# HuiGuanLab/Lite-MKD

Measured on AMD Instinct MI355X. Metric: episodes/sec (5-way 5-shot, 8x224^2 frames), higher is better.
Workload: dtype f32

## Files before the change

include/lmkd.h:

```cpp
#ifndef LMKD_H
#define LMKD_H
#ifdef __cplusplus
extern "C" {
#endif

int lmkd_abi_version(void);
const char* lmkd_last_error(void);
int lmkd_device_check(int device);
int lmkd_set_activation_dtype(int mode);
int lmkd_get_activation_dtype(void);

int lmkd_gemm_f32(char layA, char layB, int M, int N, int K, float alpha, const float* A, long lda, long sA,
                  const float* B, long ldb, long sB, float beta, float* C, long ldc, long sC, const float* bias,
                  int relu, int batch, void* stream);
int lmkd_gemm_set_mode(int mode);
int lmkd_gemm_set_tile(int t);
long lmkd_gemm_ticket_words(void);
int lmkd_gemm_f32_splitk(char layA, char layB, int M, int N, int K, float alpha, const float* A, long lda, long sA,
                         const float* B, long ldb, long sB, float beta, float* C, long ldc, long sC, const float* bias,
                         int relu, int batch, void* workspace, long ws_bytes, unsigned* tickets, void* stream);

long lmkd_conv2d_packed_weight_elems(int Cout, int Cin, int Cs, int KH, int KW, int mode);
int lmkd_conv2d_pack_weights(const float* w_oihw, float* wp, int Cout, int Cin, int Cs, int KH, int KW, int mode ,
                             void* stream);
// ... 5 lines not shown
  const void* x_words;
  const void* dy_words;
  void* out_words;
  const void* ref_words;
  int flags;
} lmkd_amax_desc;
#define LMKD_AMAX_FENCED 1
int lmkd_h2_fence_eval(const void* const* words, void* const* refs, int n, int* flags, void* stream);
long lmkd_conv_h2_fallbacks(void);
int lmkd_amax(const float* x, long n, void* word, void* stream);
long lmkd_amax_words(void);
long lmkd_conv2d_plane_elems(int ncols, int Kp);
long lmkd_conv_h2_launches(void);
int lmkd_conv2d_repack_multi(const float* const* ws, void* const* wfs, const int* dims, int n, void* stream);
int lmkd_conv2d_split_weights(const float* wp, void* wf, int ncols, int Kp, void* stream);
int lmkd_conv_get_compute_dtype(void);
int lmkd_conv_set_wgrad_planes(int on);
int lmkd_conv_set_patch(int on);
int lmkd_conv_set_stem_patch(int on);
int lmkd_conv_set_s2_patch(int on);
int lmkd_conv_set_wgrad_win16(int on);
int lmkd_conv_set_wgrad_stem(int on);
int lmkd_conv_set_wgrad_window(int on);
int lmkd_conv_set_patch16(int on);
int lmkd_conv_set_persistent(int on);
int lmkd_conv_set_xcd_mode(int mode);
int lmkd_conv_set_tile(int id);
int lmkd_conv2d_fwd(const float* x, const float* wp_fwd, float* y, float* stat_partial, int N, int H, int W, int Cs, int Cout,
                    int KH, int KW, int stride, int pad, void* stream);
int lmkd_conv2d_fwd_pre(const float* x_raw, const float* pre_stats, const float* wp_fwd, float* y, float* stat_partial, int N, int H,
                        int W, int Cs, int Cout, int KH, int KW, int stride, int pad, void* stream);
int lmkd_conv2d_fwd_bn(const float* x, const float* wp_fwd, float* y, const float* bn_stats, const float* res , int relu,
                       int N, int H, int W, int Cs, int Cout, int KH, int KW, int stride, int pad, void* stream,
                       const lmkd_amax_desc* amax );
int lmkd_conv2d_bwd_data(const float* dy, const float* wp_dgrad, float* dx, int N, int H, int W, int Cin, int Cout, int KH, int KW,
                         int stride, int pad, int accumulate, void* stream);
int lmkd_conv2d_bwd_data_bn_tiles(int N, int H, int W, int Cin, int Cout, int KH, int KW, int stride, int pad);
int lmkd_conv2d_bwd_data_bn(const float* dy, const float* wp_dgrad, float* dx, const float* bn_x, const float* bn_stats, float* part,
                            int N, int H, int W, int Cin, int Cout, int KH, int KW, int stride, int pad, void* stream);
long lmkd_conv2d_bwd_weight_workspace(int N, int H, int W, int Cs, int Cout, int KH, int KW, int stride, int pad);
int lmkd_conv2d_bwd_weight(const float* x, const float* dy, float* dw_oihw, float* workspace, long ws_bytes, int N, int H, int W,
                           int Cs, int Cin, int Cout, int KH, int KW, int stride, int pad, void* stream);
int lmkd_conv2d_bwd_weight_pre(const float* x_raw, const float* pre_stats, const float* dy, float* dw_oihw, float* workspace,
                               long ws_bytes, int N, int H, int W, int Cs, int Cin, int Cout, int KH, int KW, int stride, int pad,
                               void* stream);

// ... 236 lines not shown
```

lite-mkd_amd/_lib.py:

```python
import ctypes
import os
import re

from . import _audit

_HERE = os.path.dirname(os.path.abspath(__file__))
_ROOT = os.path.dirname(_HERE)
HEADER = os.path.join(_ROOT, "include", "lmkd.h")
LIB_PATH = os.environ.get("LMKD_LIB") or os.path.join(_HERE, "liblmkd_hip.so")

_CT = {
    "int": ctypes.c_int, "long": ctypes.c_long, "float": ctypes.c_float, "char": ctypes.c_char,
    "long long": ctypes.c_longlong, "unsigned long long": ctypes.c_ulonglong,
}


def parse_header(path=HEADER):
    txt = open(path).read()
    txt = re.sub(r"/\*.*?\*/", " ", txt, flags=re.S)
    protos = {}
    for m in re.finditer(r"\b(int|long|const char\s*\*)\s+(lmkd_\w+)\s*\(([^)]*)\)\s*;", txt):
        ret, name, args = m.group(1), m.group(2), m.group(3).strip()
        restype = ctypes.c_char_p if "char" in ret else _CT[ret]
        argtypes = []
# ... 7 lines not shown
                    ty = " ".join(toks[:-1])
                    argtypes.append(_CT[ty])
        protos[name] = (restype, argtypes)
    return protos


class _Lib:
    def __init__(self):
        if not os.path.exists(LIB_PATH):
            raise RuntimeError(
                "liblmkd_hip.so not found at %s: build it with `python lite-mkd_amd/build.py` "
                "(there is no CPU or PyTorch fallback for the hot path)" % LIB_PATH)
        import torch
        self.cdll = ctypes.CDLL(LIB_PATH)
        self.protos = parse_header()
        for name, (restype, argtypes) in self.protos.items():
            fn = getattr(self.cdll, name)
            fn.restype = restype
            fn.argtypes = argtypes
        if os.environ.get("LMKD_PATCH16"):
            self.cdll.lmkd_conv_set_patch16(int(os.environ["LMKD_PATCH16"]))
        if os.environ.get("LMKD_WGRAD_WINDOW"):
            self.cdll.lmkd_conv_set_wgrad_window(int(os.environ["LMKD_WGRAD_WINDOW"]))
        if os.environ.get("LMKD_CONV_PERSISTENT", "1") == "0":
            self.cdll.lmkd_conv_set_persistent(0)

    def last_error(self):
        return self.cdll.lmkd_last_error().decode()

    def call(self, name, *args):
        if _audit.ON:
            _audit.check(name)
        rc = getattr(self.cdll, name)(*args)
        if rc != 0:
            raise RuntimeError("%s failed (%d): %s" % (name, rc, self.last_error()))

    def value(self, name, *args):
        return getattr(self.cdll, name)(*args)


_lib = None


def lib():
    global _lib
    if _lib is None:
# ... 3 lines not shown
```

lite-mkd_amd/csrc/conv.hip:

```cpp
#include "gemm_core.h"
#include <atomic>
#include <mutex>

struct ConvGemmArgs {
  const float* src;
  const float* wpk;
  float* out;
  float* stat_partial;
  int N, Hs, Ws, Cs;
  int Hr, Wr, rows_per_class, tiles_per_class;
  int sh;
  int Ho, Wo, Co, omul;
  int Kp, cps, nclass;
  int n_rt, n_ct, xcd_mode;
  int taps_pm1;
  int grid_step;
  int grid_total;
  int same;
  int halo;
  int accum;
  const float* ep_stats;
  const float* ep_res;
  int ep_relu;
  const float* pre_stats;
// ... 1247 lines not shown
}
extern "C" int lmkd_conv2d_bwd_data_bn(const float* dy, const float* wd, float* dx, const float* bn_x, const float* bn_stats, float* part,
                                       int N, int H, int W, int Cin, int Cout, int KH, int KW, int stride, int pad, void* stream) {
  LMKD_REQUIRE(dy && wd && dx && bn_x && bn_stats && part, "lmkd_conv2d_bwd_data_bn: null pointer");
  LMKD_REQUIRE(aligned16(dy) && aligned16(wd) && aligned16(bn_x) && aligned16(bn_stats), "lmkd_conv2d_bwd_data_bn: operands must be 16-byte aligned");
  ConvGemmArgs a;
  if (const int rc = bwd_data_args(a, dy, wd, dx, N, H, W, Cin, Cout, KH, KW, stride, pad, 0)) return rc;
  a.bnb_x = bn_x; a.bnb_stats = bn_stats; a.stat_partial = part;
  const ConvPlan p = plan_dgrad(a);
  LMKD_REQUIRE(p.bnb_form, "lmkd_conv2d_bwd_data_bn: this launch has no fused form (lmkd_conv2d_bwd_data_bn_tiles returned 0)");
  return launch_conv(a, p, (hipStream_t)stream);
}

static int g_wgrad_planes = 1;
extern "C" int lmkd_conv_set_wgrad_planes(int on) { g_wgrad_planes = on ? 1 : 0; return LMKD_OK; }
static int g_wgrad_win16 = 1;
extern "C" int lmkd_conv_set_wgrad_win16(int on) { g_wgrad_win16 = on ? 1 : 0; return LMKD_OK; }
static int g_wgrad_window = 1;
extern "C" int lmkd_conv_set_wgrad_window(int on) { g_wgrad_window = on < 0 ? 0 : on; return LMKD_OK; }
static inline bool wgrad_win_eligible(int W, int Cs, int Cout, int KH, int KW, int stride, int pad) {
  return g_wgrad_window && g_wgrad_planes && conv_planes() && KH == 3 && KW == 3 && stride == 1 && pad == 1 &&
         Cs % 32 == 0 && 32 + 2 * (W + 1) <= 256;
}
static void wgrad_win_plan(int Mpix, int W, int Cs, int Cout, int* cob, int* splits, int* steps_per_split) {
  *cob = Cout >= 128 ? 4 : 2;
  const int tiles = cdiv(Cout, 32 * *cob) * (Cs / 32);
  const int steps = cdiv(Mpix, LMKD_BK);
  const int warm = cdiv(2 * (W + 1), LMKD_BK);
  const int resident = 256 * ((conv_nprod() >= 6 && *cob == 2) ? 2 : 8 / *cob);
  int sp = g_wgrad_window > 1 ? cdiv(g_wgrad_window, tiles)
                              : std::max((int)(((long)resident * steps + 19600L * 4 / *cob) / (39200L * 4 / *cob)), cdiv(128, tiles));
  const int cap = std::max(1, steps / (12 * warm));
  if (sp > cap) sp = cap;
  *steps_per_split = cdiv(steps, sp);
  *splits = cdiv(steps, *steps_per_split);
}

static void wgrad_plan(int Mpix, int Cout, int Kp, int* splits, int* steps_per_split, int* bm, int* bn, bool planes = false) {
  *bm = Cout <= 64 ? 64 : 128;
  *bn = (Kp % 128 == 0 && Kp >= 1024) ? 128 : 64;
  int per_cu = (*bm == 128 && *bn == 128) ? 2 : ((*bm == 64 && *bn == 64) ? 4 : 3);
  if (planes) {
    if (*bm == 64 && *bn == 128) *bn = 64;
    const int npl = conv_nprod() == 1 ? 1 : 3;
    const long lds = 1L * npl * LMKD_BK * ((*bm * 2 + 64) + (*bn * 2 + 64));
    per_cu = (int)(160 * 1024 / lds);
    if (per_cu > 4) per_cu = 4;
    if (per_cu < 1) per_cu = 1;
  }
  const int tiles = cdiv(Cout, *bm) * cdiv(Kp, *bn);
  const int steps = cdiv(Mpix, LMKD_BK);
  const int slots = 256 * per_cu;
  int best_sp = 1;
  double best_cost = 1e30;
// ... 14 lines not shown

static int g_wgrad_stem = 1;
extern "C" int lmkd_conv_set_wgrad_stem(int on) { g_wgrad_stem = on ? 1 : 0; return LMKD_OK; }
static int stem_wgrad_plan(int N, int H, int W, int Cs, int Cout, int KH, int KW, int stride, int pad, int* G) {
  if (!g_wgrad_stem || !g_wgrad_planes || conv_nprod(g_lmkd_act_bf16) < 6 || Cs != 4 || Cout != 64 || KH != 7 || KW != 7 || stride != 2 || pad != 3) return 0;
  const int Ho = conv_out(H, KH, stride, pad), Wo = conv_out(W, KW, stride, pad);
  if (Wo < 17 || Wo > 128 || W > 2 * Wo || Ho < 1) return 0;
  const int units = N * cdiv(Ho, 2);
  int g = std::max(1, 2048 / (2 * Wo));
  g = std::min(g, std::max(1, units / 256));
  *G = g;
  return cdiv(units, g);
}

enum class WgFam : unsigned char {
  Stem,
  Win16,
  Win,
  Planes,
  Tile,
};
struct WgradPlan {
  WgFam fam;
  bool pre, act16, smallc;
  int nprod;
  int bm, bn;
  int cob;
  int G;
  int splits, splits0, sps0, sps1, seg_pix0;
  int xcd;
  int grid;
  long need;
  long ws;
};

static long wgrad_workspace(int N, int H, int W, int Cs, int Cout, int KH, int KW, int stride, int pad) {
  const int Ho = conv_out(H, KH, stride, pad), Wo = conv_out(W, KW, stride, pad);
  const int Kp = KH * kw_padded(Cs, KW) * Cs;
  int G, splits, sps, bm, bn;
  if (const int slabs = stem_wgrad_plan(N, H, W, Cs, Cout, KH, KW, stride, pad, &G)) return (long)slabs * Cout * Kp * sizeof(float);
  wgrad_plan(N * Ho * Wo, Cout, Kp, &splits, &sps, &bm, &bn, conv_planes() && g_wgrad_planes);
  if (wgrad_win_eligible(W, Cs, Cout, KH, KW, stride, pad)) {
    int cob, wsplits, wsps;
    wgrad_win_plan(N * Ho * Wo, W, Cs, Cout, &cob, &wsplits, &wsps);
    splits = std::max(splits, wsplits);
  }
  return (long)splits * Cout * Kp * sizeof(float);
}

static WgradPlan plan_wgrad(int N, int H, int W, int Cs, int Cout, int KH, int KW, int stride, int pad, int seg_n0, bool pre, bool maxima) {
  WgradPlan p;
  memset(&p, 0, sizeof(p));
  const bool act16 = g_lmkd_act_bf16;
  const int Ho = conv_out(H, KH, stride, pad), Wo = conv_out(W, KW, stride, pad);
  const int Kp = KH * kw_padded(Cs, KW) * Cs, Mpix = N * Ho * Wo;
  p.pre = pre; p.act16 = act16; p.smallc = Cs == 4;
  p.ws = wgrad_workspace(N, H, W, Cs, Cout, KH, KW, stride, pad);
  if (seg_n0)
    p.ws = std::max(p.ws, wgrad_workspace(seg_n0, H, W, Cs, Cout, KH, KW, stride, pad) + wgrad_workspace(N - seg_n0, H, W, Cs, Cout, KH, KW, stride, pad));
  p.seg_pix0 = seg_n0 ? seg_n0 * Ho * Wo : Mpix;
  if (const int slabs = stem_wgrad_plan(N, H, W, Cs, Cout, KH, KW, stride, pad, &p.G)) {
    p.fam = WgFam::Stem;
    p.nprod = conv_nprod(false, maxima);
    p.splits = p.grid = slabs;
  } else if (wgrad_win_eligible(W, Cs, Cout, KH, KW, stride, pad)) {
    const bool w16 = g_wgrad_win16 && conv_nprod(act16) >= 6;
    p.fam = w16 ? WgFam::Win16 : WgFam::Win;
    p.nprod = w16 ? conv_nprod(false, maxima) : conv_nprod(act16);
    wgrad_win_plan(Mpix, W, Cs, Cout, &p.cob, &p.splits, &p.sps0);
    p.splits0 = p.splits;
    if (seg_n0) {
      int sp1, cob1;
      wgrad_win_plan(p.seg_pix0, W, Cs, Cout, &p.cob, &p.splits0, &p.sps0);
      wgrad_win_plan(Mpix - p.seg_pix0, W, Cs, Cout, &cob1, &sp1, &p.sps1);
      p.splits = p.splits0 + sp1;
    }
    p.grid = 8 * cdiv(p.splits, 8) * cdiv(Cout, 32 * p.cob) * (Cs / 32);
  } else {
    const bool planes = conv_planes() && g_wgrad_planes;
    p.fam = planes ? WgFam::Planes : WgFam::Tile;
    p.nprod = planes ? conv_nprod(act16, maxima && !p.smallc && !pre) : (conv_nprod() == 1 ? 1 : 0);
    wgrad_plan(Mpix, Cout, Kp, &p.splits, &p.sps0, &p.bm, &p.bn, planes);
    p.splits0 = p.splits;
    if (seg_n0) {
      int sp1, bm1, bn1;
      wgrad_plan(p.seg_pix0, Cout, Kp, &p.splits0, &p.sps0, &p.bm, &p.bn, planes);
      wgrad_plan(Mpix - p.seg_pix0, Cout, Kp, &sp1, &p.sps1, &bm1, &bn1, planes);
      p.splits = p.splits0 + sp1;
    }
    p.xcd = (g_xcd_mode != 0 && g_xcd_mode != 1 && p.splits >= 32) ? 1 : 0;
    p.grid = (p.xcd ? 8 * cdiv(p.splits, 8) : p.splits) * cdiv(Cout, p.bm) * cdiv(Kp, p.bn);
  }
  p.need = (long)p.splits * Cout * Kp * sizeof(float);
  return p;
}

template <int NPROD, int D, int RLC>
static void launch_stem_wgrad(const StemWgradArgs& w, dim3 grid, size_t lds, hipStream_t s) {
  lds_attr_once<stem_wgrad_kernel<NPROD, D, RLC>>(160 * 1024);
  hipLaunchKernelGGL((stem_wgrad_kernel<NPROD, D, RLC>), grid, dim3(512), lds, s, w);
}
template <int NPROD>
static void launch_stem_wgrad(const StemWgradArgs& w, dim3 grid, size_t lds, hipStream_t s) {
  const bool deep = cdiv(2 * w.Wo, 32) >= 6;
  if (deep && w.RL == 1856) launch_stem_wgrad<NPROD, 6, 1856>(w, grid, lds, s);
  else if (deep) launch_stem_wgrad<NPROD, 6, 0>(w, grid, lds, s);
  else launch_stem_wgrad<NPROD, 2, 0>(w, grid, lds, s);
}
template <int COB>
static void launch_wgrad_win(const WgradWinArgs& w, const WgradPlan& p, bool big, hipStream_t s) {
  const dim3 grid(p.grid);
  if (p.fam == WgFam::Win16) {
    constexpr int JW = COB == 2 ? 1 : 2;
    constexpr int NT = 64 * COB * (2 / JW);
    with_nprod<3, 6, 9>(p.nprod, [&](auto np) {
      if (big && p.pre) hipLaunchKernelGGL((conv_wgrad_win16_kernel<COB, np, 256, true, 9, JW>), grid, dim3(NT), 0, s, w);
      else if (big) hipLaunchKernelGGL((conv_wgrad_win16_kernel<COB, np, 256, false, 9, JW>), grid, dim3(NT), 0, s, w);
      else if (p.pre) hipLaunchKernelGGL((conv_wgrad_win16_kernel<COB, np, 128, true, 9, JW>), grid, dim3(NT), 0, s, w);
      else hipLaunchKernelGGL((conv_wgrad_win16_kernel<COB, np, 128, false, 9, JW>), grid, dim3(NT), 0, s, w);
    });
    return;
  }
  auto go = [&](auto np, auto a16, auto pre) {
    constexpr int NPROD = decltype(np)::value;
    constexpr bool A16 = decltype(a16)::value, PRE = decltype(pre)::value;
    constexpr int TPW = (COB == 2 && NPROD != 1) ? 5 : 9;
    constexpr int NT = 64 * COB * ((9 + TPW - 1) / TPW);
    if (big) hipLaunchKernelGGL((conv_wgrad_win_kernel<COB, NPROD, A16, 256, PRE, TPW>), grid, dim3(NT), 0, s, w);
    else hipLaunchKernelGGL((conv_wgrad_win_kernel<COB, NPROD, A16, 128, PRE, TPW>), grid, dim3(NT), 0, s, w);
  };
  using T = std::true_type;
  using F = std::false_type;
  if (p.act16) go(std::integral_constant<int, 1>{}, T{}, F{});
  else with_nprod<1, 6, 9>(p.nprod, [&](auto np) { if (p.pre) go(np, F{}, T{}); else go(np, F{}, F{}); });
// ... 46 lines not shown
  if (p.fam == WgFam::Stem) {
    LMKD_REQUIRE((long)Mpix * 64 * 4 < 0xffffffe0L && (long)N * H * W * 16 < 0xffffffe0L, "lmkd_conv2d_bwd_weight: tensor too large for 32-bit byte offsets");
    StemWgradArgs w;
    memset(&w, 0, sizeof(w));
    w.dy = dy; w.x = x; w.slab = workspace;
    w.h2_xw = amax_x; w.h2_dyw = amax_dy;
    w.N = N; w.H = H; w.W = W; w.Ho = Ho; w.Wo = Wo;
    w.upi = cdiv(Ho, 2); w.units = N * w.upi; w.G = p.G; w.slabs = p.splits;
    w.RL = 16 * Wo + 64;
    const size_t lds = (size_t)2 * 10 * 3 * w.RL + 2 * 3 * STEM_WG_APLANE;
    with_nprod<3, 6, 9>(p.nprod, [&](auto np) { launch_stem_wgrad<np>(w, dim3(p.grid), lds, s); });
    LMKD_CHECK_LAUNCH("stem_wgrad_kernel");
    if (Kp <= 256) {
      hipLaunchKernelGGL(wgrad_reduce_stem_kernel, dim3(Cout), dim3(256, 4), 0, s, (const float*)workspace, dw_oihw, p.splits, Cout, Cin, Cs, KH, KW,
                         KWp, Kp, accumulate);
    } else {
      launch_wgrad_reduce((const float*)workspace, dw_oihw, p.splits, Cout, Cin, Cs, KH, KW, KWp, Kp, accumulate, s);
    }
    LMKD_CHECK_LAUNCH("wgrad_reduce_kernel");
    return LMKD_OK;
  }
  if (p.fam == WgFam::Win16 || p.fam == WgFam::Win) {
    LMKD_REQUIRE((long)Mpix * std::max(Cs, Cout) * 4 < 2147483647L, "lmkd_conv2d_bwd_weight: tensor too large for 32-bit byte offsets");
    WgradWinArgs w;
    memset(&w, 0, sizeof(w));
    w.dy = dy; w.x = x; w.slab = workspace; w.pre_stats = pre_stats;
    w.h2_xw = amax_x; w.h2_dyw = amax_dy;
    w.N = N; w.H = H; w.W = W; w.Cs = Cs; w.Co = Cout; w.Kp = Kp; w.Mpix = Mpix;
    w.steps_total = cdiv(Mpix, LMKD_BK);
    w.splits = p.splits; w.steps_per_split = p.sps0;
    w.seg_pix0 = p.seg_pix0; w.seg_splits0 = p.splits0; w.sps1 = p.sps1;
    w.n_ct = cdiv(Cout, 32 * p.cob); w.n_it = Cs / 32;
    w.div_hw = make_fastdiv(H * W); w.div_w = make_fastdiv(W);
    const bool big = 32 + 2 * (W + 1) > 128;
    if (p.cob == 4) launch_wgrad_win<4>(w, p, big, s);
    else launch_wgrad_win<2>(w, p, big, s);
    LMKD_CHECK_LAUNCH("conv_wgrad_win_kernel");
    launch_wgrad_reduce((const float*)workspace, dw_oihw, p.splits, Cout, Cin, Cs, KH, KW, KWp, Kp, accumulate, s);
    LMKD_CHECK_LAUNCH("wgrad_reduce_kernel");
    return LMKD_OK;
  }
  WgradArgs a;
  memset(&a, 0, sizeof(a));
  a.dy = dy; a.x = x; a.slab = workspace; a.pre_stats = pre_stats;
  a.h2_xw = amax_x; a.h2_dyw = amax_dy;
  a.N = N; a.Hs = H; a.Ws = W; a.Cs = Cs;
  a.Ho = Ho; a.Wo = Wo; a.Co = Cout;
  a.stride = stride; a.pad = pad; a.KH = KH; a.KW = KW; a.KWp = KWp;
  a.Kp = Kp; a.Mpix = Mpix;
  a.steps_per_split = p.sps0;
  a.seg_pix0 = p.seg_pix0; a.seg_splits0 = p.splits0; a.sps1 = p.sps1;
  a.steps_total = cdiv(Mpix, LMKD_BK);
  a.div_hw = make_fastdiv(Ho * Wo); a.div_w = make_fastdiv(Wo);
  a.n_mt = cdiv(Cout, p.bm); a.n_jt = cdiv(Kp, p.bn); a.splits = p.splits;
  a.xcd_mode = p.xcd;
  const int bm = p.bm, bn = p.bn;
// ... 40 lines not shown
extern "C" int lmkd_conv2d_bwd_weight_acc(const float* x, const float* pre_stats, const float* dy, float* dw_oihw, float* workspace,
                                          long ws_bytes, int N, int H, int W, int Cs, int Cin, int Cout, int KH, int KW, int stride,
                                          int pad, void* stream) {
  return conv2d_bwd_weight_impl(x, pre_stats, dy, dw_oihw, workspace, ws_bytes, N, H, W, Cs, Cin, Cout, KH, KW, stride, pad, stream, 1);
}


extern "C" int lmkd_conv2d_bwd_weight_seg(const float* x, const float* pre_stats, const float* dy, float* dw_oihw, float* workspace, long ws_bytes,
                                          int N, int H, int W, int Cs, int Cin, int Cout, int KH, int KW, int stride, int pad, int accumulate,
                                          int seg_n0, void* stream, const lmkd_amax_desc* amax) {
  return conv2d_bwd_weight_impl(x, pre_stats, dy, dw_oihw, workspace, ws_bytes, N, H, W, Cs, Cin, Cout, KH, KW, stride, pad, stream, accumulate, seg_n0, amax);
}

extern "C" int lmkd_conv2d_plan(int kind, int N, int H, int W, int Cs, int Cin, int Cout, int KH, int KW, int stride, int pad,
                                int* info) {
  LMKD_REQUIRE(info && kind >= 0 && kind <= 2, "lmkd_conv2d_plan: kind must be 0 (forward), 1 (data gradient) or 2 (weight gradient)");
  LMKD_REQUIRE(N > 0 && H > 0 && W > 0 && Cout > 0 && KH > 0 && KW > 0 && stride > 0, "lmkd_conv2d_plan: bad shape");
  if (kind == 2) {
    const WgradPlan p = plan_wgrad(N, H, W, Cs, Cout, KH, KW, stride, pad, 0, false, false);
    info[1] = p.xcd; info[2] = p.splits; info[3] = p.grid;
    switch (p.fam) {
      case WgFam::Stem: info[0] = 14; info[4] = 2; break;
      case WgFam::Win16:
      case WgFam::Win: info[0] = p.cob == 4 ? 5 : 6; info[1] = 1; info[4] = 1; break;
      default: info[0] = (p.bm == 128 && p.bn == 128) ? 1 : (p.bm == 128 ? 2 : (p.bn == 128 ? 4 : 3)); info[4] = 0; break;
    }
    return LMKD_OK;
  }
  ConvGemmArgs a;
  if (kind == 0) fwd_geometry(a, N, H, W, Cs, Cout, KH, KW, stride, pad, 0);
  else dgrad_geometry(a, N, H, W, Cin, Cout, KH, KW, stride, pad, 0);
  const ConvPlan p = kind == 0 ? plan_fwd(a, KH, KW, pad) : plan_dgrad(a);
  info[0] = p.tile; info[1] = p.xcd; info[2] = p.nclass; info[3] = p.grid;
  info[4] = p.fam == ConvFam::Stem ? 2 : (p.fam == ConvFam::Patch || p.fam == ConvFam::Patch16 || p.fam == ConvFam::Patch1p ? 1 : 0);
  return LMKD_OK;
}
```

lite-mkd_amd/csrc/wgrad_win.h:

```cpp
#pragma once

struct WgradWinArgs {
  const float* dy;
  const float* x;
  float* slab;
  const float* pre_stats;
  int N, H, W, Cs, Co, Kp;
  int Mpix, steps_total, steps_per_split, splits;
  int n_ct, n_it;
  int seg_pix0, seg_splits0, sps1;
  FastDiv div_hw, div_w;
  const unsigned* h2_xw;
  const unsigned* h2_dyw;
};
template <int COB, int NPROD, bool ACT16, int R, bool PRE = false, int TPW = 9>
__global__ __launch_bounds__(64 * COB * ((9 + TPW - 1) / TPW)) void conv_wgrad_win_kernel(WgradWinArgs a) {
  constexpr int NPL = NPROD == 1 ? 1 : 3;
  static_assert(!ACT16 || (NPROD == 1 && !PRE), "bf16 tensors: one plane, no store-side arithmetic");
  constexpr int THREADS = 64 * COB * ((9 + TPW - 1) / TPW), BM = 32 * COB;
  constexpr int LDA = BM * 2 + 64, A_PLANE = LMKD_BK * LDA;
  constexpr int LDX = 64, X_PLANE = (R + 1) * LDX;
  constexpr int ESZ = ACT16 ? 2 : 4, EPL = ACT16 ? 8 : 4;
  constexpr int A_LPR = BM / EPL, A_RPP = THREADS / A_LPR, A_NI = (LMKD_BK + A_RPP - 1) / A_RPP;
  constexpr int X_LPR = 32 / EPL, X_RPP = THREADS / X_LPR, X_NI = (LMKD_BK + X_RPP - 1) / X_RPP;
// ... 150 lines not shown
            c = __builtin_amdgcn_mfma_f32_32x32x16_bf16(fa[g][1], fb[0], c, 0, 0, 0);
            c = __builtin_amdgcn_mfma_f32_32x32x16_bf16(fa[g][0], fb[0], c, 0, 0, 0);
          }
        }
        acc[ti] = c;
      }
      __syncthreads();
    }
  }

  float* C = a.slab + (long)z * a.Co * a.Kp;
#pragma unroll
  for (int ti = 0; ti < TPW; ++ti) {
    if (9 % TPW != 0 && tap0 + ti >= 9) break;
    const int col = (tap0 + ti) * a.Cs + ci0 + (lane & 31);
#pragma unroll
    for (int e = 0; e < 16; ++e) {
      const int row = co0 + cw * 32 + acc_row(e, lane);
      if (row < a.Co) C[(long)row * a.Kp + col] = acc[ti][e];
    }
  }
}

template <int COB, int NPROD, int R, bool PRE = false, int TPW = 9, int JW = 2>
__global__ __launch_bounds__(64 * COB * ((9 + TPW - 1) / TPW) * (2 / JW), JW == 2 ? 2 : 3) void conv_wgrad_win16_kernel(WgradWinArgs a) {
  static_assert(JW == 2 || (JW == 1 && TPW == 9), "the channel-block split exists for nine taps per wave");
  static_assert(NPROD == 6 || NPROD == 9 || NPROD == 3, "three bf16 planes (6 / 9 products) or two fp16 planes (3 products: conv_patch16.h)");
  constexpr int NPL = NPROD == 3 ? 2 : 3;
  constexpr int THREADS = 64 * COB * ((9 + TPW - 1) / TPW) * (2 / JW), BM = 32 * COB;
  constexpr int LDA = BM * 2 + 32, A_PLANE = LMKD_BK * LDA;
  constexpr int LDX = 64, X_PLANE = (R + 1) * LDX;
  constexpr int A_LPR = BM / 4, A_RPP = THREADS / A_LPR, A_NI = (LMKD_BK + A_RPP - 1) / A_RPP;
  constexpr int X_LPR = 8, X_RPP = THREADS / X_LPR, X_NI = (LMKD_BK + X_RPP - 1) / X_RPP;
  static_assert(THREADS % A_LPR == 0 && THREADS % X_LPR == 0 && (LDA / 32) % 2 == 1, "tile layout");
  __shared__ __attribute__((aligned(16))) unsigned char s_dy[NPL * A_PLANE];
  __shared__ __attribute__((aligned(16))) unsigned char s_x[NPL * X_PLANE];
  __shared__ __attribute__((aligned(16))) unsigned s_adr[2][9 * LMKD_BK];
  const int tid = threadIdx.x, lane = tid & 63, wave = tid >> 6;
  const int tiles = a.n_ct * a.n_it;
  const int xj = blockIdx.x >> 3;
  const int z = (blockIdx.x & 7) + 8 * (xj / tiles);
  if (z >= a.splits) return;
  const int tz = xj - (xj / tiles) * tiles;
  const int co0 = (tz % a.n_ct) * BM, ci0 = (tz / a.n_ct) * 32;
  const WinSlab sl = win_slab(z, a.Mpix, a.steps_per_split, a.seg_pix0, a.seg_splits0, a.sps1);
  const int nk = sl.nk, kend = sl.kend;
  const int halo = a.W + 1;

  const __amdgpu_buffer_rsrc_t rs_dy = x3_rsrc(a.dy, (long)a.Mpix * a.Co * 4);
  const __amdgpu_buffer_rsrc_t rs_x = x3_rsrc(a.x, (long)a.Mpix * a.Cs * 4);
  const int a_c = (tid % A_LPR) * 4, a_r = tid / A_LPR;
  const bool a_cin = co0 + a_c < a.Co;
  const int x_c = (tid % X_LPR) * 4, x_r = tid / X_LPR;
  u32x4 ra[A_NI], rx[X_NI];
  unsigned x_ok = 0;
  float h2_sx = 1.f, h2_sdy = 1.f;
  if constexpr (NPROD == 3) {
    h2_sx = h2_scale(amax_read(a.h2_xw, sl.seg));
    h2_sdy = h2_scale(amax_read(a.h2_dyw, sl.seg));
  }
  float4 psc = float4(), psh = float4();
  if (PRE) {
    psc = *reinterpret_cast<const float4*>(a.pre_stats + (long)sl.seg * 5 * a.Cs + 2 * a.Cs + ci0 + x_c);
    psh = *reinterpret_cast<const float4*>(a.pre_stats + (long)sl.seg * 5 * a.Cs + 3 * a.Cs + ci0 + x_c);
  }
  auto load_dy = [&](int k0) {
#pragma unroll
    for (int i = 0; i < A_NI; ++i) {
      const int p = k0 + a_r + A_RPP * i;
      ra[i] = __builtin_amdgcn_raw_buffer_load_b128(rs_dy, (a_cin && a_r + A_RPP * i < LMKD_BK && p < kend) ? (unsigned)((p * a.Co + co0 + a_c) * 4) : X3_OOB, 0, 0);
    }
  };
  auto load_x = [&](int q0) {
#pragma unroll
    for (int i = 0; i < X_NI; ++i) {
      const int q = q0 + x_r + X_RPP * i;
      const bool ok = x_r + X_RPP * i < LMKD_BK && q >= 0 && q < a.Mpix;
      rx[i] = __builtin_amdgcn_raw_buffer_load_b128(rs_x, ok ? (unsigned)((q * a.Cs + ci0 + x_c) * 4) : X3_OOB, 0, 0);
      if (PRE) x_ok = ok ? (x_ok | (1u << i)) : (x_ok & ~(1u << i));
    }
  };
  auto as_f4 = [](const u32x4& r) { return make_float4(__uint_as_float(r.x), __uint_as_float(r.y), __uint_as_float(r.z), __uint_as_float(r.w)); };
  auto store_dy = [&]() {
#pragma unroll
    for (int i = 0; i < A_NI; ++i) {
      if (a_r + A_RPP * i >= LMKD_BK) continue;
      if constexpr (NPROD == 3) {
        uint2 p0, p1;
        h2_split4(as_f4(ra[i]), h2_sdy, p0, p1);
        unsigned char* d = s_dy + (a_r + A_RPP * i) * LDA + a_c * 2;
        *reinterpret_cast<uint2*>(d) = p0;
        *reinterpret_cast<uint2*>(d + A_PLANE) = p1;
      } else {
        tr_store4<NPL, LDA, A_PLANE>(s_dy, a_r + A_RPP * i, a_c, as_f4(ra[i]));
      }
    }
  };
  auto store_x = [&](int q0) {
#pragma unroll
    for (int i = 0; i < X_NI; ++i) {
      if (x_r + X_RPP * i >= LMKD_BK) continue;
      const int slot = (q0 + x_r + X_RPP * i) & (R - 1);
      float4 v = as_f4(rx[i]);
      if (PRE && ((x_ok >> i) & 1u)) {
        v.x = fmaxf(fmaf(v.x, psc.x, psh.x), 0.f); v.y = fmaxf(fmaf(v.y, psc.y, psh.y), 0.f);
        v.z = fmaxf(fmaf(v.z, psc.z, psh.z), 0.f); v.w = fmaxf(fmaf(v.w, psc.w, psh.w), 0.f);
      }
      uint2 p0, p1, p2;
      if constexpr (NPROD == 3) h2_split4(v, h2_sx, p0, p1); else x3_split4(v, p0, p1, p2);
      unsigned char* d = s_x + slot * LDX + ((x_c * 2) ^ (((slot >> 2) & 1) << 5));
      *reinterpret_cast<uint2*>(d) = p0;
      *reinterpret_cast<uint2*>(d + X_PLANE) = p1;
      if constexpr (NPL == 3) *reinterpret_cast<uint2*>(d + 2 * X_PLANE) = p2;
    }
  };
  auto fill_adr = [&](unsigned* tab, int k0) {
    for (int e = tid; e < 9 * LMKD_BK; e += THREADS) {
      const int tp = e >> 5, r = e & 31;
      const int p = k0 + r;
      unsigned adr = (unsigned)(R * LDX);
      if (p < kend) {
        const int n = fdiv(p, a.div_hw);
        const int rem = p - n * a.H * a.W;
        const int h = fdiv(rem, a.div_w), w = rem - h * a.W;
        const int dh = tp / 3 - 1, dw = tp - (tp / 3) * 3 - 1;
        if ((unsigned)(h + dh) < (unsigned)a.H && (unsigned)(w + dw) < (unsigned)a.W) {
          const int slot = (p + dh * a.W + dw) & (R - 1);
          adr = (unsigned)(slot * LDX + (((slot >> 2) & 1) << 5));
        }
      }
      tab[tp * LMKD_BK + (r & 15) * 2 + (r >> 4)] = adr;
    }
  };

  const int q4 = lane >> 4, idx = lane & 15;
  const int cw = wave % COB, tap0 = JW == 2 ? (wave / COB) * TPW : 0, j0 = JW == 2 ? 0 : wave / COB;
  const int offA = (4 * q4 + (idx >> 2)) * LDA + (cw * 32 + 4 * (idx & 3)) * 2;
  const unsigned cbx = (unsigned)(8 * (idx & 3));
  f32x4 acc[TPW][2][JW];
#pragma unroll
  for (int t = 0; t < TPW; ++t)
#pragma unroll
    for (int i = 0; i < 2; ++i)
#pragma unroll
      for (int j = 0; j < JW; ++j) acc[t][i][j] = f32x4{0.f, 0.f, 0.f, 0.f};

  if (nk > 0) {
    const int kfirst = sl.kfirst;
    for (int j = tid; j < NPL * LDX / 4; j += THREADS)
      reinterpret_cast<unsigned*>(s_x + (j / (LDX / 4)) * X_PLANE + R * LDX)[j % (LDX / 4)] = 0u;
    for (int q0 = kfirst - halo; q0 < kfirst + halo; q0 += LMKD_BK) {
      load_x(q0);
      store_x(q0);
    }
    fill_adr(s_adr[0], kfirst);
    load_dy(kfirst);
    load_x(kfirst + halo);
    for (int t = 0; t < nk; ++t) {
      const int k0 = kfirst + t * LMKD_BK;
      store_dy();
      store_x(k0 + halo);
      __syncthreads();
      if (t + 1 < nk) {
        load_dy(k0 + LMKD_BK);
        load_x(k0 + LMKD_BK + halo);
        fill_adr(s_adr[(t + 1) & 1], k0 + LMKD_BK);
      }
      bf16x8 fa[2][NPL];
#pragma unroll
      for (int i = 0; i < 2; ++i)
#pragma unroll
        for (int p = 0; p < NPL; ++p) {
          const unsigned char* ap = s_dy + p * A_PLANE + offA + i * 32;
          const s16x4_t lo = __builtin_amdgcn_ds_read_tr16_b64_v4i16((s16x4_t __attribute__((address_space(3)))*)ap);
          const s16x4_t hi = __builtin_amdgcn_ds_read_tr16_b64_v4i16((s16x4_t __attribute__((address_space(3)))*)(ap + 16 * LDA));
          union { s16x4_t s[2]; bf16x8 b; } u;
          u.s[0] = lo; u.s[1] = hi;
          fa[i][p] = u.b;
        }
      if constexpr (NPROD == 3 && JW == 2) {
        static_assert(NPROD != 3 || TPW == 9, "all nine taps per wave");
        auto read_fb = [&](int tp, bf16x8 (&fb)[JW][NPL]) {
          const uint2 a2 = *reinterpret_cast<const uint2*>(&s_adr[t & 1][tp * LMKD_BK + (4 * q4 + (idx >> 2)) * 2]);
#pragma unroll
          for (int j = 0; j < JW; ++j) {
            const unsigned lo_a = (a2.x ^ (unsigned)((j0 + j) << 5)) + cbx, hi_a = (a2.y ^ (unsigned)((j0 + j) << 5)) + cbx;
#pragma unroll
            for (int p = 0; p < NPL; ++p) {
// ... 67 lines not shown
              c = __builtin_amdgcn_mfma_f32_16x16x32_f16(__builtin_bit_cast(f16x8, fa[i][1]), __builtin_bit_cast(f16x8, fb[0]), c, 0, 0, 0);
              c = __builtin_amdgcn_mfma_f32_16x16x32_f16(__builtin_bit_cast(f16x8, fa[i][0]), __builtin_bit_cast(f16x8, fb[1]), c, 0, 0, 0);
              c = __builtin_amdgcn_mfma_f32_16x16x32_f16(__builtin_bit_cast(f16x8, fa[i][0]), __builtin_bit_cast(f16x8, fb[0]), c, 0, 0, 0);
              acc[ti][i][j] = c;
              continue;
            }
            if (NPROD == 9) {
              c = __builtin_amdgcn_mfma_f32_16x16x32_bf16(fa[i][NPL - 1], fb[NPL - 1], c, 0, 0, 0);
              c = __builtin_amdgcn_mfma_f32_16x16x32_bf16(fa[i][1], fb[NPL - 1], c, 0, 0, 0);
              c = __builtin_amdgcn_mfma_f32_16x16x32_bf16(fa[i][NPL - 1], fb[1], c, 0, 0, 0);
            }
            c = __builtin_amdgcn_mfma_f32_16x16x32_bf16(fa[i][1], fb[1], c, 0, 0, 0);
            c = __builtin_amdgcn_mfma_f32_16x16x32_bf16(fa[i][0], fb[NPL - 1], c, 0, 0, 0);
            c = __builtin_amdgcn_mfma_f32_16x16x32_bf16(fa[i][NPL - 1], fb[0], c, 0, 0, 0);
            c = __builtin_amdgcn_mfma_f32_16x16x32_bf16(fa[i][0], fb[1], c, 0, 0, 0);
            c = __builtin_amdgcn_mfma_f32_16x16x32_bf16(fa[i][1], fb[0], c, 0, 0, 0);
            c = __builtin_amdgcn_mfma_f32_16x16x32_bf16(fa[i][0], fb[0], c, 0, 0, 0);
            acc[ti][i][j] = c;
          }
        }
      }
      __syncthreads();
    }
  }

  float* C = a.slab + (long)z * a.Co * a.Kp;
  const float h2_ix = 1.f / h2_sx, h2_idy = 1.f / h2_sdy;
#pragma unroll
  for (int ti = 0; ti < TPW; ++ti) {
    if (9 % TPW != 0 && tap0 + ti >= 9) break;
#pragma unroll
    for (int i = 0; i < 2; ++i)
#pragma unroll
      for (int j = 0; j < JW; ++j) {
        const int col = (tap0 + ti) * a.Cs + ci0 + 16 * (j0 + j) + idx;
#pragma unroll
        for (int e = 0; e < 4; ++e) {
          const int row = co0 + cw * 32 + 16 * i + 4 * q4 + e;
          if (row < a.Co) C[(long)row * a.Kp + col] = NPROD == 3 ? acc[ti][i][j][e] * h2_ix * h2_idy : acc[ti][i][j][e];
        }
      }
  }
}
```

Before: 49.54.

## Add windowed LDS weight-gradient kernel for stride-2 3x3 convolutions

Extends the windowed Win16 weight-gradient path to stride-2, pad-1 3x3 convolutions. Input pixels are loaded as four phase rings indexed by output position, and the tap address table maps each tap to a ring slot. This lets stride-2 layers reuse the sliding-window LDS scheme instead of the generic GEMM path. The split planning is adjusted for stride 2. The change also adds an env toggle, an LDS-size query and optional timing stamps, and it costs more LDS for the four rings.

```diff
diff --git a/include/lmkd.h b/include/lmkd.h
--- a/include/lmkd.h
+++ b/include/lmkd.h
@@ -51,6 +51,8 @@
 int lmkd_conv_set_wgrad_win16(int on);
 int lmkd_conv_set_wgrad_stem(int on);
 int lmkd_conv_set_wgrad_window(int on);
+int lmkd_conv_set_wgrad_s2_window(int on);
+int lmkd_conv2d_bwd_weight_s2_window_lds(int H, int W, int Cs, int Cout, int maxima);
 int lmkd_conv_set_patch16(int on);
 int lmkd_conv_set_persistent(int on);
 int lmkd_conv_set_xcd_mode(int mode);
diff --git a/lite-mkd_amd/_lib.py b/lite-mkd_amd/_lib.py
--- a/lite-mkd_amd/_lib.py
+++ b/lite-mkd_amd/_lib.py
@@ -53,6 +53,8 @@
             self.cdll.lmkd_conv_set_patch16(int(os.environ["LMKD_PATCH16"]))
         if os.environ.get("LMKD_WGRAD_WINDOW"):
             self.cdll.lmkd_conv_set_wgrad_window(int(os.environ["LMKD_WGRAD_WINDOW"]))
+        if os.environ.get("LMKD_WGRAD_S2_WIN", "1") == "0":
+            self.cdll.lmkd_conv_set_wgrad_s2_window(0)
         if os.environ.get("LMKD_CONV_PERSISTENT", "1") == "0":
             self.cdll.lmkd_conv_set_persistent(0)
 
diff --git a/lite-mkd_amd/csrc/conv.hip b/lite-mkd_amd/csrc/conv.hip
--- a/lite-mkd_amd/csrc/conv.hip
+++ b/lite-mkd_amd/csrc/conv.hip
@@ -1293,14 +1293,25 @@
   return g_wgrad_window && g_wgrad_planes && conv_planes() && KH == 3 && KW == 3 && stride == 1 && pad == 1 &&
          Cs % 32 == 0 && 32 + 2 * (W + 1) <= 256;
 }
-static void wgrad_win_plan(int Mpix, int W, int Cs, int Cout, int* cob, int* splits, int* steps_per_split) {
+static int g_wgrad_s2_win = 1;
+extern "C" int lmkd_conv_set_wgrad_s2_window(int on) { g_wgrad_s2_win = on ? 1 : 0; return LMKD_OK; }
+static inline bool wgrad_win_s2_eligible(int H, int W, int Cs, int Cout, int KH, int KW, int stride, int pad, bool pre) {
+  return g_wgrad_s2_win && g_wgrad_window && g_wgrad_planes && g_wgrad_win16 && conv_nprod(g_lmkd_act_bf16) == 6 && KH == 3 && KW == 3 &&
+         stride == 2 && pad == 1 && H % 2 == 0 && W % 2 == 0 && Cs % 32 == 0 && Cout >= 128 && W / 2 + 1 <= LMKD_BK;
+}
+extern "C" int lmkd_conv2d_bwd_weight_s2_window_lds(int H, int W, int Cs, int Cout, int maxima) {
+  if (!wgrad_win_s2_eligible(H, W, Cs, Cout, 3, 3, 2, 1, false)) return 0;
+  return win16_lds_bytes(4, conv_nprod(false, maxima != 0) == 3 ? 2 : 3, 64, true);
+}
+static void wgrad_win_plan(int Mpix, int W, int Cs, int Cout, int* cob, int* splits, int* steps_per_split, bool s2 = false, int hw = 0) {
   *cob = Cout >= 128 ? 4 : 2;
   const int tiles = cdiv(Cout, 32 * *cob) * (Cs / 32);
   const int steps = cdiv(Mpix, LMKD_BK);
-  const int warm = cdiv(2 * (W + 1), LMKD_BK);
+  const int warm = s2 ? cdiv(W + 1, LMKD_BK) : cdiv(2 * (W + 1), LMKD_BK);
   const int resident = 256 * ((conv_nprod() >= 6 && *cob == 2) ? 2 : 8 / *cob);
+  const long episode = s2 ? (long)cdiv(400 * hw, LMKD_BK) * tiles : 39200L * 4 / *cob;
   int sp = g_wgrad_window > 1 ? cdiv(g_wgrad_window, tiles)
-                              : std::max((int)(((long)resident * steps + 19600L * 4 / *cob) / (39200L * 4 / *cob)), cdiv(128, tiles));
+                              : std::max((int)(((long)resident * steps + episode / 2) / episode), cdiv(128, tiles));
   const int cap = std::max(1, steps / (12 * warm));
   if (sp > cap) sp = cap;
   *steps_per_split = cdiv(steps, sp);
@@ -1361,7 +1372,7 @@
 };
 struct WgradPlan {
   WgFam fam;
-  bool pre, act16, smallc;
+  bool pre, act16, smallc, s2;
   int nprod;
   int bm, bn;
   int cob;
@@ -1382,6 +1393,10 @@
   if (wgrad_win_eligible(W, Cs, Cout, KH, KW, stride, pad)) {
     int cob, wsplits, wsps;
     wgrad_win_plan(N * Ho * Wo, W, Cs, Cout, &cob, &wsplits, &wsps);
+    splits = std::max(splits, wsplits);
+  } else if (wgrad_win_s2_eligible(H, W, Cs, Cout, KH, KW, stride, pad, false)) {
+    int cob, wsplits, wsps;
+    wgrad_win_plan(N * Ho * Wo, Wo, Cs, Cout, &cob, &wsplits, &wsps, true, Ho * Wo);
     splits = std::max(splits, wsplits);
   }
   return (long)splits * Cout * Kp * sizeof(float);
@@ -1402,16 +1417,17 @@
     p.fam = WgFam::Stem;
     p.nprod = conv_nprod(false, maxima);
     p.splits = p.grid = slabs;
-  } else if (wgrad_win_eligible(W, Cs, Cout, KH, KW, stride, pad)) {
+  } else if ((p.s2 = wgrad_win_s2_eligible(H, W, Cs, Cout, KH, KW, stride, pad, pre)) || wgrad_win_eligible(W, Cs, Cout, KH, KW, stride, pad)) {
     const bool w16 = g_wgrad_win16 && conv_nprod(act16) >= 6;
+    const int Ww = p.s2 ? Wo : W;
     p.fam = w16 ? WgFam::Win16 : WgFam::Win;
     p.nprod = w16 ? conv_nprod(false, maxima) : conv_nprod(act16);
-    wgrad_win_plan(Mpix, W, Cs, Cout, &p.cob, &p.splits, &p.sps0);
+    wgrad_win_plan(Mpix, Ww, Cs, Cout, &p.cob, &p.splits, &p.sps0, p.s2, Ho * Wo);
     p.splits0 = p.splits;
     if (seg_n0) {
       int sp1, cob1;
-      wgrad_win_plan(p.seg_pix0, W, Cs, Cout, &p.cob, &p.splits0, &p.sps0);
-      wgrad_win_plan(Mpix - p.seg_pix0, W, Cs, Cout, &cob1, &sp1, &p.sps1);
+      wgrad_win_plan(p.seg_pix0, Ww, Cs, Cout, &p.cob, &p.splits0, &p.sps0, p.s2, Ho * Wo);
+      wgrad_win_plan(Mpix - p.seg_pix0, Ww, Cs, Cout, &cob1, &sp1, &p.sps1, p.s2, Ho * Wo);
       p.splits = p.splits0 + sp1;
     }
     p.grid = 8 * cdiv(p.splits, 8) * cdiv(Cout, 32 * p.cob) * (Cs / 32);
@@ -1449,6 +1465,14 @@
 template <int COB>
 static void launch_wgrad_win(const WgradWinArgs& w, const WgradPlan& p, bool big, hipStream_t s) {
   const dim3 grid(p.grid);
+  if (p.s2) {
+    if constexpr (COB == 4)
+      with_nprod<3, 6>(p.nprod, [&](auto np) {
+        if (p.pre) hipLaunchKernelGGL((conv_wgrad_win16_kernel<4, np, 64, true, 9, 2, true>), grid, dim3(256), 0, s, w);
+        else hipLaunchKernelGGL((conv_wgrad_win16_kernel<4, np, 64, false, 9, 2, true>), grid, dim3(256), 0, s, w);
+      });
+    return;
+  }
   if (p.fam == WgFam::Win16) {
     constexpr int JW = COB == 2 ? 1 : 2;
     constexpr int NT = 64 * COB * (2 / JW);
@@ -1541,6 +1565,7 @@
   }
   if (p.fam == WgFam::Win16 || p.fam == WgFam::Win) {
     LMKD_REQUIRE((long)Mpix * std::max(Cs, Cout) * 4 < 2147483647L, "lmkd_conv2d_bwd_weight: tensor too large for 32-bit byte offsets");
+    LMKD_REQUIRE(!p.s2 || ((long)N * H * W * Cs * 4 < 0xffffffe0L && p.cob == 4), "lmkd_conv2d_bwd_weight: tensor too large for 32-bit byte offsets");
     WgradWinArgs w;
     memset(&w, 0, sizeof(w));
     w.dy = dy; w.x = x; w.slab = workspace; w.pre_stats = pre_stats;
@@ -1551,6 +1576,10 @@
     w.seg_pix0 = p.seg_pix0; w.seg_splits0 = p.splits0; w.sps1 = p.sps1;
     w.n_ct = cdiv(Cout, 32 * p.cob); w.n_it = Cs / 32;
     w.div_hw = make_fastdiv(H * W); w.div_w = make_fastdiv(W);
+    if (p.s2) {
+      w.H = Ho; w.W = Wo;
+      w.div_hw = make_fastdiv(Ho * Wo); w.div_w = make_fastdiv(Wo);
+    }
     const bool big = 32 + 2 * (W + 1) > 128;
     if (p.cob == 4) launch_wgrad_win<4>(w, p, big, s);
     else launch_wgrad_win<2>(w, p, big, s);
@@ -1637,7 +1666,7 @@
     switch (p.fam) {
       case WgFam::Stem: info[0] = 14; info[4] = 2; break;
       case WgFam::Win16:
-      case WgFam::Win: info[0] = p.cob == 4 ? 5 : 6; info[1] = 1; info[4] = 1; break;
+      case WgFam::Win: info[0] = p.cob == 4 ? 5 : 6; info[1] = 1; info[4] = p.s2 ? 3 : 1; break;
       default: info[0] = (p.bm == 128 && p.bn == 128) ? 1 : (p.bm == 128 ? 2 : (p.bn == 128 ? 4 : 3)); info[4] = 0; break;
     }
     return LMKD_OK;
diff --git a/lite-mkd_amd/csrc/wgrad_win.h b/lite-mkd_amd/csrc/wgrad_win.h
--- a/lite-mkd_amd/csrc/wgrad_win.h
+++ b/lite-mkd_amd/csrc/wgrad_win.h
@@ -196,17 +196,30 @@
   }
 }
 
-template <int COB, int NPROD, int R, bool PRE = false, int TPW = 9, int JW = 2>
+#ifdef LMKD_STAMPS
+#define WSTAMPV(k, v) do { if (threadIdx.x == 0 && (blockIdx.x & 63) == 0 && (blockIdx.x >> 6) < 4096) g_lmkd_stamps[(blockIdx.x >> 6) * 8 + (k)] = (v); } while (0)
+#else
+#define WSTAMPV(k, v) do { } while (0)
+#endif
+constexpr int win16_lds_bytes(int cob, int npl, int r, bool s2) {
+  return npl * LMKD_BK * (32 * cob * 2 + 32) + npl * ((s2 ? 4 : 1) * r + 1) * 64 + 2 * 9 * LMKD_BK * 4;
+}
+template <int COB, int NPROD, int R, bool PRE = false, int TPW = 9, int JW = 2, bool S2 = false>
 __global__ __launch_bounds__(64 * COB * ((9 + TPW - 1) / TPW) * (2 / JW), JW == 2 ? 2 : 3) void conv_wgrad_win16_kernel(WgradWinArgs a) {
+  static_assert(!S2 || (TPW == 9 && JW == 2 && COB == 4 && R == 64 && NPROD != 9), "stride 2: the four-wave, nine-tap instance");
   static_assert(JW == 2 || (JW == 1 && TPW == 9), "the channel-block split exists for nine taps per wave");
   static_assert(NPROD == 6 || NPROD == 9 || NPROD == 3, "three bf16 planes (6 / 9 products) or two fp16 planes (3 products: conv_patch16.h)");
   constexpr int NPL = NPROD == 3 ? 2 : 3;
   constexpr int THREADS = 64 * COB * ((9 + TPW - 1) / TPW) * (2 / JW), BM = 32 * COB;
   constexpr int LDA = BM * 2 + 32, A_PLANE = LMKD_BK * LDA;
-  constexpr int LDX = 64, X_PLANE = (R + 1) * LDX;
+  constexpr int NR = S2 ? 4 : 1;
+  constexpr int LDX = 64, X_PLANE = (NR * R + 1) * LDX;
   constexpr int A_LPR = BM / 4, A_RPP = THREADS / A_LPR, A_NI = (LMKD_BK + A_RPP - 1) / A_RPP;
   constexpr int X_LPR = 8, X_RPP = THREADS / X_LPR, X_NI = (LMKD_BK + X_RPP - 1) / X_RPP;
+  constexpr int X_NL = S2 ? 4 : X_NI;
   static_assert(THREADS % A_LPR == 0 && THREADS % X_LPR == 0 && (LDA / 32) % 2 == 1, "tile layout");
+  static_assert(!S2 || X_NI == 1, "stride 2: one pixel row per thread and step");
+  static_assert(NPL * A_PLANE + NPL * X_PLANE + 2 * 9 * LMKD_BK * 4 == win16_lds_bytes(COB, NPL, R, S2), "win16_lds_bytes");
   __shared__ __attribute__((aligned(16))) unsigned char s_dy[NPL * A_PLANE];
   __shared__ __attribute__((aligned(16))) unsigned char s_x[NPL * X_PLANE];
   __shared__ __attribute__((aligned(16))) unsigned s_adr[2][9 * LMKD_BK];
@@ -220,13 +233,14 @@
   const WinSlab sl = win_slab(z, a.Mpix, a.steps_per_split, a.seg_pix0, a.seg_splits0, a.sps1);
   const int nk = sl.nk, kend = sl.kend;
   const int halo = a.W + 1;
+  STAMP(0);
 
   const __amdgpu_buffer_rsrc_t rs_dy = x3_rsrc(a.dy, (long)a.Mpix * a.Co * 4);
-  const __amdgpu_buffer_rsrc_t rs_x = x3_rsrc(a.x, (long)a.Mpix * a.Cs * 4);
+  const __amdgpu_buffer_rsrc_t rs_x = x3_rsrc(a.x, (long)a.Mpix * a.Cs * 4 * NR);
   const int a_c = (tid % A_LPR) * 4, a_r = tid / A_LPR;
   const bool a_cin = co0 + a_c < a.Co;
   const int x_c = (tid % X_LPR) * 4, x_r = tid / X_LPR;
-  u32x4 ra[A_NI], rx[X_NI];
+  u32x4 ra[A_NI], rx[X_NL];
   unsigned x_ok = 0;
   float h2_sx = 1.f, h2_sdy = 1.f;
   if constexpr (NPROD == 3) {
@@ -245,7 +259,24 @@
       ra[i] = __builtin_amdgcn_raw_buffer_load_b128(rs_dy, (a_cin && a_r + A_RPP * i < LMKD_BK && p < kend) ? (unsigned)((p * a.Co + co0 + a_c) * 4) : X3_OOB, 0, 0);
     }
   };
-  auto load_x = [&](int q0) {
+  auto load_x = [&](int q0, bool warm = false) {
+    if constexpr (S2) {
+      const int q = q0 + x_r;
+      const bool ok = q >= 0 && q < a.Mpix;
+      if (PRE) x_ok = ok ? 1u : 0u;
+      const int qq = ok ? q : 0;
+      const int n = fdiv(qq, a.div_hw);
+      const int rem = qq - n * a.H * a.W;
+      const int oh = fdiv(rem, a.div_w), ow = rem - oh * a.W;
+      const unsigned src = (unsigned)((((n * 2 * a.H + 2 * oh) * 2 * a.W + 2 * ow) * a.Cs + ci0 + x_c) * 4);
+#pragma unroll
+      for (int c = 0; c < 4; ++c) {
+        if (c == 3 && warm) continue;
+        const int ph = 1 - (c >> 1), pw = 1 - (c & 1);
+        rx[c] = __builtin_amdgcn_raw_buffer_load_b128(rs_x, ok ? src + (unsigned)((ph * 2 * a.W + pw) * a.Cs * 4) : X3_OOB, 0, 0);
+      }
+      return;
+    }
 #pragma unroll
     for (int i = 0; i < X_NI; ++i) {
       const int q = q0 + x_r + X_RPP * i;
@@ -270,7 +301,26 @@
       }
     }
   };
-  auto store_x = [&](int q0) {
+  auto store_x = [&](int q0, bool warm = false) {
+    if constexpr (S2) {
+      const int slot = (q0 + x_r) & (R - 1);
+#pragma unroll
+      for (int c = 0; c < 4; ++c) {
+        if (c == 3 && warm) continue;
+        float4 v = as_f4(rx[c]);
+        if (PRE && (x_ok & 1u)) {
+          v.x = fmaxf(fmaf(v.x, psc.x, psh.x), 0.f); v.y = fmaxf(fmaf(v.y, psc.y, psh.y), 0.f);
+          v.z = fmaxf(fmaf(v.z, psc.z, psh.z), 0.f); v.w = fmaxf(fmaf(v.w, psc.w, psh.w), 0.f);
+        }
+        uint2 p0, p1, p2;
+        if constexpr (NPROD == 3) h2_split4(v, h2_sx, p0, p1); else x3_split4(v, p0, p1, p2);
+        unsigned char* d = s_x + (c * R + slot) * LDX + ((x_c * 2) ^ (((slot >> 2) & 1) << 5));
+        *reinterpret_cast<uint2*>(d) = p0;
+        *reinterpret_cast<uint2*>(d + X_PLANE) = p1;
+        if constexpr (NPL == 3) *reinterpret_cast<uint2*>(d + 2 * X_PLANE) = p2;
+      }
+      return;
+    }
 #pragma unroll
     for (int i = 0; i < X_NI; ++i) {
       if (x_r + X_RPP * i >= LMKD_BK) continue;
@@ -292,15 +342,24 @@
     for (int e = tid; e < 9 * LMKD_BK; e += THREADS) {
       const int tp = e >> 5, r = e & 31;
       const int p = k0 + r;
-      unsigned adr = (unsigned)(R * LDX);
+      unsigned adr = (unsigned)(NR * R * LDX);
       if (p < kend) {
         const int n = fdiv(p, a.div_hw);
         const int rem = p - n * a.H * a.W;
         const int h = fdiv(rem, a.div_w), w = rem - h * a.W;
+        if constexpr (S2) {
+          const int kh = tp / 3, kw = tp - kh * 3;
+          const int dh = kh == 0 ? -1 : 0, dw = kw == 0 ? -1 : 0;
+          if (h + dh >= 0 && w + dw >= 0) {
+            const int ring = 2 * (kh == 1) + (kw == 1), slot = (p + dh * a.W + dw) & (R - 1);
+            adr = (unsigned)((ring * R + slot) * LDX + (((slot >> 2) & 1) << 5));
+          }
+        } else {
         const int dh = tp / 3 - 1, dw = tp - (tp / 3) * 3 - 1;
         if ((unsigned)(h + dh) < (unsigned)a.H && (unsigned)(w + dw) < (unsigned)a.W) {
           const int slot = (p + dh * a.W + dw) & (R - 1);
           adr = (unsigned)(slot * LDX + (((slot >> 2) & 1) << 5));
+        }
         }
       }
       tab[tp * LMKD_BK + (r & 15) * 2 + (r >> 4)] = adr;
@@ -322,22 +381,37 @@
   if (nk > 0) {
     const int kfirst = sl.kfirst;
     for (int j = tid; j < NPL * LDX / 4; j += THREADS)
-      reinterpret_cast<unsigned*>(s_x + (j / (LDX / 4)) * X_PLANE + R * LDX)[j % (LDX / 4)] = 0u;
+      reinterpret_cast<unsigned*>(s_x + (j / (LDX / 4)) * X_PLANE + NR * R * LDX)[j % (LDX / 4)] = 0u;
+    const int ahead = S2 ? 0 : halo;
+    if constexpr (S2) {
+      load_x(kfirst - LMKD_BK, true);
+      store_x(kfirst - LMKD_BK, true);
+    } else
     for (int q0 = kfirst - halo; q0 < kfirst + halo; q0 += LMKD_BK) {
       load_x(q0);
       store_x(q0);
     }
     fill_adr(s_adr[0], kfirst);
     load_dy(kfirst);
-    load_x(kfirst + halo);
+    load_x(kfirst + ahead);
+    STAMP(1);
+#ifdef LMKD_STAMPS
+    unsigned long long st_fill = 0;
+#endif
     for (int t = 0; t < nk; ++t) {
       const int k0 = kfirst + t * LMKD_BK;
+#ifdef LMKD_STAMPS
+      const unsigned long long st_t = __builtin_amdgcn_s_memtime();
+#endif
       store_dy();
-      store_x(k0 + halo);
+      store_x(k0 + ahead);
       __syncthreads();
+#ifdef LMKD_STAMPS
+      st_fill += __builtin_amdgcn_s_memtime() - st_t;
+#endif
       if (t + 1 < nk) {
         load_dy(k0 + LMKD_BK);
-        load_x(k0 + LMKD_BK + halo);
+        load_x(k0 + LMKD_BK + ahead);
         fill_adr(s_adr[(t + 1) & 1], k0 + LMKD_BK);
       }
       bf16x8 fa[2][NPL];
@@ -451,6 +525,11 @@
       }
       __syncthreads();
     }
+    STAMP(2);
+#ifdef LMKD_STAMPS
+    WSTAMPV(4, st_fill);
+    WSTAMPV(5, (unsigned long long)nk);
+#endif
   }
 
   float* C = a.slab + (long)z * a.Co * a.Kp;
@@ -470,4 +549,5 @@
         }
       }
   }
+  STAMP(3);
 }
```

Measured after the change: 49.92, median of 6. No clear change (+0.8%).
